# FAST-ASR/MarkovModels.jl

Measured on AMD Instinct MI355X. Metric: pdfposteriors_frames_per_sec, higher is better.
Workload: dtype f32

## Files before the change

### markovmodels.jl_amd/csrc/mm_engine.hip

```cpp
#include <hip/hip_runtime.h>
#include <dlfcn.h>

#include <algorithm>
#include <atomic>
#include <cmath>
#include <cstdio>
#include <cstdlib>
#include <chrono>
#include <cstring>
#include <limits>
#include <new>
#include <map>
#include <memory>
#include <mutex>
#include <string>
#include <thread>
#include <vector>

#include "../../include/markovmodels_amd.h"
#include "mm_kernels.hip"
#include "mm_kernel_quad.hip"
#include "mm_kernel_rows.hip"
#include "mm_internal.h"
#include "mm_pack.h"
// ... 2248 lines not shown
            "32-bit values), mm_stream_combine_kernel, mm_stream_finish_kernel, then for marked utterances only " + redo;
    case Fb::Split: {
        const std::string k = std::to_string(mm_pair_nj(h->max_P1, h->pair_H)), H = std::to_string(h->pair_H);
        return "mm_fbs_kernel<" + k + ",A," + H + ">, then <" + k + ",B," + H + "> (forward and backward agents in one grid, teams of " + H +
            " workgroups), mm_pair_finish_kernel, then for marked utterances only " +
            (h->dpair_ok ? "mm_fbds_kernel<" + k + ",A," + H + ">, then <" + k + ",B," + H + "> (float64, one utterance per team" +
                               (h->wpair_ok ? std::string("); FIRST and alone while the inputs are hard: mm_fbws_kernel<") + k + ",A," + H + ">, then <" + k +
                                                  ",B," + H + "> (wide-exponent pairs, two utterances per team)"
                                            : std::string("; FIRST and alone while the inputs are hard)")) +
                               ", mm_dpair_finish_kernel, then for what those mark "
                         : std::string()) +
            pair_tail;
    }
    case Fb::Pairs: {
        const std::string k = std::to_string(mm_pair_nj(h->max_P1));
        return "mm_fbp_kernel<" + k + ",A>, then <" + k + ",B> (forward and backward agents in one grid), mm_pair_finish_kernel, then for marked "
            "utterances only " +
            (h->dpair_ok ? "mm_fbd_kernel<" + k + ",A>, then <" + k + ",B> (float64, one utterance per workgroup" +
                               (h->wpair_ok ? std::string("); FIRST and alone while the inputs are hard: mm_fbw_kernel<") + k + ",A>, then <" + k +
                                                  ",B> (wide-exponent pairs, two utterances per workgroup)"
                                            : std::string("; FIRST and alone while the inputs are hard)")) +
                               ", mm_dpair_finish_kernel, then for what those mark "
                         : std::string()) +
            pair_tail;
    }
    case Fb::Rows: {
        auto ka = [&](int d) {
            for (int k : kRowKA)
                if (h->row_ka[d] <= k) return k;
            return 0;
        };
        return "mm_fbr_kernel<" + std::to_string(ka(0)) + ",8192,0> + mm_fbr_kernel<" + std::to_string(ka(1)) +
// ... 48 lines not shown
        const std::string inst = "<" + std::to_string(pl.NI) + "," + where_of(pl.global) + ">";
        s = "mm_leaky_fwd_kernel" + inst + " (forward: alpha~ with the leak term in the row epilogue) + mm_leaky_bwd_kernel" + inst +
            " (backward: z, then beta = z (+) eps c, gamma per pdf); state vectors " + (pl.global ? "in global memory" : "in LDS");
    } else if (entry == 2) {
        s = h->gen.last_kernels.empty() ? std::string("mm_generic_kernel (not called yet)") : h->gen.last_kernels;
    } else {
        return fail(MM_ERR_INVALID, "mm_batch_kernels: unknown entry");
    }
    snprintf(buf, n, "%s", s.c_str());
    return MM_OK;
}

static size_t ws_c_bytes(mm_batch_t h, int64_t N) { return align_up(size_t(h->B + 1) * size_t(N + 2) * 8, 256); }

struct WsLayout {
    size_t alpha = 0, c = 0, order = 0, redo = 0, hand = 0, zmin = 0, x = 0, x_rows = 0, xd = 0, xd_rows = 0, redo2 = 0;
    size_t extra = 0, em_max = 0, stream[4] = {0, 0, 0, 0}, total = 0;
};

static WsLayout ws_layout(mm_batch_t h, int64_t N) {
    WsLayout L;
    const size_t B = size_t(h->B), marks = align_up((B + 1) * 4, 256);
    L.c = on_pairs(h) ? align_up((B + 1) * size_t(h->pair_H > 1 ? h->split_s1p : h->max_S1p) * size_t(N + 2) * 4 + 16384, 256)
                      : align_up(size_t(h->total_s1p) * size_t(N + 1) * 4, 256);
    L.order = L.c + ws_c_bytes(h, N);
    L.redo = L.order + marks;
    L.hand = L.redo + marks;
    L.zmin = L.hand + align_up((B + 1) * 2 * mm_pair_hand_bytes(), 256);
    L.x = L.zmin + align_up(B * 6 * 8, 256);
    L.xd = L.redo2 = L.x;
    if (h->pair_H > 1) {
        const size_t H = size_t(h->pair_H), row = 2 * size_t(h->split_s1p) * 4, xps = size_t(mm_pair_xps(h->max_P1, h->pair_H)) * 4;
        L.x_rows = 2 * ((B + 1) / 2) * 2 * H * 2 * row;
        L.xd = L.redo2 = L.x + align_up(L.x_rows + ((B + 1) / 2) * 2 * H * 4 * xps, 256);
        if (h->dpair_ok) {
            L.xd_rows = 2 * B * 2 * H * 2 * row;
            L.redo2 = L.xd + align_up(L.xd_rows + B * 2 * H * 4 * xps + 65536, 256);
        }
    }
    L.extra = L.redo2 + marks;
    L.total = L.extra;
    if (h->fb == Fb::Stream) {
        L.total += mm_stream_extra_bytes(h->B, h->total_s1p, N, L.stream, h->stream_H, h->stream_S1);
        for (size_t &o : L.stream) o += L.extra;
// ... 194 lines not shown
        }
    }
    return launch_log<MODE_FB>(h, p, stream);
}

static int fb_linear(mm_batch_t h, RunParams &p, char *ws, const WsLayout &L, bool exact_first, void *stream) {
    h->last_redo = p.redo;
    h->last_exact_first = exact_first;
    int rc;
    if (h->fb == Fb::Rows) {
        rc = launch_rows(h, p, stream);
    } else {
        p.pair_s1p = h->pair_H > 1 ? h->split_s1p : h->max_S1p;
        p.pair_hand = ws + L.hand;
        p.pair_zmin = reinterpret_cast<double *>(ws + L.zmin);
        if (h->fb == Fb::Split) {
            p.xbuf_d = reinterpret_cast<float *>(ws + L.xd);
            p.xps_d = reinterpret_cast<float *>(ws + L.xd + L.xd_rows);
            p.x_phase_d = (long long)(L.xd_rows / 8);
            p.x_H = h->dpair_ok ? h->pair_H : 0;
            rc = bind_team_x(h, p, ws, L, exact_first, stream);
            if (rc) return rc;
        }
        h->last_z = p.pair_zmin;
        rc = exact_first ? MM_OK : launch_pairs(h, p, stream);
    }
    if (rc) return rc;
    if (h->dbg.no_redo && !exact_first) return MM_OK;
    if (h->dpair_ok) {
        const PairLaunch pl = pair_launch_of(h);
// ... 43 lines not shown
        if (h->dpair_ok) {
            const int64_t M = h->stat_host[0], H = h->pair_H, cus = std::max(1, h->n_cus);
            auto rounds = [&](int64_t wgs) { return (wgs + cus - 1) / cus; };
            const bool by_rounds = M > 0 && (h->wpair_ok || rounds(2 * h->B * H) <= rounds(2 * ((h->B + 1) / 2) * H) + rounds(2 * std::min<int64_t>(M, h->B) * H));
            exact_first = h->exact_first >= 0 ? h->exact_first != 0 : (by_rounds && !capturing(stream));
            p.redo2 = reinterpret_cast<int *>(ws + L.redo2);
            p.stat_dev = h->stat_dev;
            p.stat_xcd = h->xcd_counting ? 1 : 0;
            p.stat_host = h->stat_host;
            p.stat_seq = ++h->stat_seq;
            p.stat_mode = exact_first ? 1 : 0;
        }
    }
    if (ordered || marks) {
        hipLaunchKernelGGL(mm_prologue_kernel, dim3(unsigned((h->B + 1 + 255) / 256)), dim3(256), 0, static_cast<hipStream_t>(stream),
                           lens, int(h->B), int(N), order, p.redo, p.redo2, exact_first ? 1 : 0);
        HIP_TRY(hipGetLastError());
    }
    bind_stamps(h, p);
    switch (h->fb) {
    case Fb::Lane: return fb_lane(h, p, ws, L, stream);
    case Fb::Stream: return fb_stream(h, p, ws, L, stream);
    case Fb::Wave: return fb_wave(h, p, ws, L, stream);
    case Fb::Rows:
    case Fb::Pairs:
    case Fb::Split: return fb_linear(h, p, ws, L, exact_first, stream);
    case Fb::Quad:
    case Fb::Item: break;
    }
    return fb_exact(h, p, ws, L, stream);
}
// ... 344 lines not shown
        const WsLayout L = ws_layout(h, N);
        rc = ensure_ws(h, L.total, stream);
        if (rc) return rc;
        char *const ws = static_cast<char *>(h->ws);
        p.ws_alpha = reinterpret_cast<float *>(ws + L.alpha);
        p.ws_c = reinterpret_cast<double *>(ws + L.c);
        p.redo = reinterpret_cast<int *>(ws + L.redo);
        p.pair_s1p = h->pair_H > 1 ? h->split_s1p : h->max_S1p;
        p.pair_hand = ws + L.hand;
        p.pair_zmin = reinterpret_cast<double *>(ws + L.zmin);
        p.split_q10 = 512;
        p.lt_floor = h->lt_floor;
        p.x_sleep = h->dbg.x_sleep;
        p.x_timeout = x_timeout(N);
        hipLaunchKernelGGL(mm_prologue_kernel, dim3(unsigned((h->B + 1 + 255) / 256)), dim3(256), 0, static_cast<hipStream_t>(stream),
                           (const int *)nullptr, int(h->B), int(N), (int *)nullptr, p.redo, (int *)nullptr, 0);
        HIP_TRY(hipGetLastError());
        if (h->pair_H > 1) {
            rc = bind_team_x(h, p, ws, L, false, stream);
            if (rc) return rc;
            rc = mm_launch_split_export(pair_launch_of(h), p, mode == MODE_ALPHA ? 0 : 1, static_cast<hipStream_t>(stream));
        } else {
            rc = mm_launch_pair_export(pair_launch_of(h), p, mode == MODE_ALPHA ? 0 : 1, static_cast<hipStream_t>(stream));
        }
        if (rc) return rc;
        if (h->stat_host) {
            hipLaunchKernelGGL(mm_count_marks_kernel, dim3(1), dim3(256), 0, static_cast<hipStream_t>(stream), p.redo, int(h->B),
                               const_cast<int *>(h->stat_host) + 2 + (mode == MODE_ALPHA ? 0 : 1));
            HIP_TRY(hipGetLastError());
        }
        h->last_redo = p.redo;
// ... 173 lines not shown
```

### markovmodels.jl_amd/csrc/mm_kernel_dpair.hip

```cpp
#pragma once
#include "mm_kernel_pairs.hip"

namespace mm {

__device__ __forceinline__ double ldsr_d(unsigned addr) { return *(__attribute__((address_space(3))) const double *)(__UINTPTR_TYPE__)addr; }
__device__ __forceinline__ void ldsw_d(unsigned addr, double v) { *(__attribute__((address_space(3))) double *)(__UINTPTR_TYPE__)addr = v; }

__device__ __forceinline__ double dexp2(float y) {
    float fl = __builtin_floorf(y);
    fl = __builtin_fmaxf(fl, -1100.f);
    const float m = fast_exp2(y - fl);
    return __builtin_amdgcn_ldexp((double)m, (int)fl);
}
__device__ __forceinline__ float dlog2(double s) {
    const int ex = __builtin_amdgcn_frexp_exp(s);
    const float mf = (float)__builtin_amdgcn_frexp_mant(s);
    return (float)ex + fast_log2(mf);
}

#ifndef MM_DPAIR_LINFIN
#define MM_DPAIR_LINFIN 1
#endif
#define MM_DLINF_EMIN (-500.f)
template <int NJ>
// ... 857 lines not shown
            if (t1 > t0)
                dpair_pdf_sums<(NJ > 4 ? 1 : (NJ > 2 ? 2 : 3))>(L::Q(t1 & 1), L::PDFSE, L::PSUM(t1 & 1), P1, wave, NWC, lane, H > 1 ? xps_send + (t1 & 3) * (int)L::XPS : nullptr,
                               H > 1 && split_tag(t1, t0, 2) != 0u);
            __syncthreads();
        }
    }
#ifdef MM_STAMPS
    if (p.dbg && lane == 0 && H == 1)
        for (int k = 0; k < 2; ++k) p.dbg[(((long long)ui * MM_MAX_WAVES + wave) * 4 + PHASE * 2 + DIR) * 2 + k] = stamp_acc[k];
#endif
}

static __global__ void mm_dpair_finish_kernel(RunParams p) {
    const int b = blockIdx.x;
    if (p.redo[b] == 0) {
        if (p.stat_mode == 1 && threadIdx.x == 0) report_hard(p, 0);
        return;
    }
    int len = p.lens ? p.lens[b] : p.N;
    len = len < 0 ? 0 : (len > p.N ? p.N : len);
    const int P = p.utts[b].P1 - 1;
    if (threadIdx.x == 0) {
        const double z0 = p.pair_zmin[6 * b], z1 = p.pair_zmin[6 * b + 1];
        const double z = z0 < z1 ? z0 : z1;
        const double y0 = p.pair_zmin[6 * b + 2], y1 = p.pair_zmin[6 * b + 3];
        const double zM = y0 > y1 ? y0 : y1;
        const double l0 = p.pair_zmin[6 * b + 4], l1 = p.pair_zmin[6 * b + 5];
        const double lm = l0 < l1 ? l0 : l1;
        p.ttl[b] = (z < __builtin_inf()) ? (float)(z * (double)MM_LN2) : MM_NINF;
        const bool agree = z > -__builtin_inf() && zM < __builtin_inf() && zM - z <= MM_Z_SPREAD_TOL;
        if (p.redo2[b] == 1 && agree && lm >= (double)p.lt_floor - (double)MM_DPAIR_THR_EXTRA) p.redo2[b] = 0;
        if (p.redo2[b] == 0 && len >= 1 && !(zM < __builtin_inf())) p.redo2[b] = 1;
        if (p.redo2[b] == 0 && len >= 1 && !(z == -__builtin_inf() && zM == -__builtin_inf()) && !(lm >= (double)p.lt_floor - (double)MM_DPAIR_THR_EXTRA)) p.redo2[b] = 1;
        if (p.stat_mode == 1) report_hard(p, !(lm >= (double)p.lt_floor));
    }
    const long long gbase = (long long)b * p.gsb;
    for (long long q = threadIdx.x; q < (long long)(p.N - len) * P; q += blockDim.x)
        p.gamma[gbase + (len + q / P) * p.gsn + (q % P) * p.gsp] = 0.f;
}

}
```

### markovmodels.jl_amd/csrc/mm_kernel_pairs.hip

```cpp
#pragma once
#include <algorithm>
#include "mm_internal.h"
#include "mm_kernel_rows.hip"

namespace mm {

typedef float mm_f32x2 __attribute__((ext_vector_type(2)));
typedef unsigned mm_u32x2 __attribute__((ext_vector_type(2)));
__device__ __forceinline__ mm_u32x2 ldsr2u(unsigned addr) { return *(__attribute__((address_space(3))) const mm_u32x2 *)(__UINTPTR_TYPE__)addr; }
__device__ __forceinline__ mm_f32x2 ldsr2(unsigned addr) { return *(__attribute__((address_space(3))) const mm_f32x2 *)(__UINTPTR_TYPE__)addr; }
__device__ __forceinline__ void ldsw2(unsigned addr, float a, float b) {
    mm_f32x2 v = {a, b};
    *(__attribute__((address_space(3))) mm_f32x2 *)(__UINTPTR_TYPE__)addr = v;
}

constexpr int pair_pc(int NJ) { return NJ > 4 ? 64 * NJ : 256; }
constexpr int pair_nr(int RS, int PC) { return (PC > 256 || RS > 16384) ? 2 : 3; }
template <int RS, int PHASE, int RSH = 2 * RS, int PC = 256>
struct PairLay {
    static constexpr unsigned RS2 = 2 * RS;
    static constexpr unsigned PC4 = 4u * PC, PC8 = 8u * PC;
    static constexpr int NR = pair_nr(RS, PC);
    static constexpr unsigned RAWS = 2u * PC4;
    static constexpr unsigned XPS = 2u * PC;
// ... 614 lines not shown
    M(0) M(2) M(4) M(6) MM_PAIR_PRIO(MM_PAIR_PRIO_A, 1) M(8) M(10) M(12)                                     \
    if (lastp >= 14) {                                                                                       \
        M(14) MM_PAIR_PRIO(MM_PAIR_PRIO_B, 0) M(16)                                                          \
        if (lastp >= 18) {                                                                                   \
            M(18)                                                                                            \
            if (lastp >= 20) { M(20) M(22) }                                                                 \
        }                                                                                                    \
    }

struct PairHand {
    float m_prev, s_cur, s_prev, cbar;
    int seen, pad;
    double cum;
};

template <int KA, int RS, int PHASE, int DIRT, int NJ, int H = 1, int RSH = 2 * RS, bool SMALL = false, bool XPT = false>
__device__ __forceinline__ void pair_agent(const RunParams &p, int pair, int hset = 0, int rdir = 0) {
#ifndef MM_SPLIT_MAXTRACK
#define MM_SPLIT_MAXTRACK 0
#endif
    extern __shared__ float lds[];
    const int DIR = DIRT < 0 ? __builtin_amdgcn_readfirstlane(rdir) : DIRT;
    const unsigned long long x_tmo = p.x_timeout;
    using L = PairLay<RS, PHASE, RSH, pair_pc(NJ)>;
#ifndef MM_PAIR_DA
#define MM_PAIR_DA 3
#endif
#ifndef MM_PAIR_DB
#define MM_PAIR_DB 3
#endif
#ifndef MM_PAIR_EXITS_B
#define MM_PAIR_EXITS_B 1
// ... 30 lines not shown
    float *rowsP = p.ws_alpha + (long long)pair * (long long)(p.N + 2) * 2 * p.pair_s1p;
    const UttDesc &ud = p.utts[U[0].b];
    const RowU r = uni(H > 1 ? ud.rps[DIR][hset] : ud.rp[DIR]);
    const int S1 = r.rows, S1p = p.pair_s1p, P1 = uni(ud.P1), P = P1 - 1, P1p = (P1 + 3) & ~3;
    const float thr = r.thr;
    unsigned sthr = 0u;
    if constexpr (LINF && !ADAPT)
        asm volatile("v_readfirstlane_b32 %0, %1" : "=s"(sthr) : "v"(((unsigned)(127 - (int)(thr + MM_LINF_EMIN < 1.f ? 1.f : thr + MM_LINF_EMIN)) << 23) - 1u));
    int m = (int)(((long long)NFp * (p.split_q10 > 0 ? p.split_q10 : 512)) >> 10);
    m = m < 1 ? 1 : (m > NFp - 1 && NFp > 1 ? NFp - 1 : m);
    const int tA = XPT ? NFp : (DIR ? NFp - m : m), tEnd = NFp;
    auto frame_of = [&](int t) { return DIR ? NFp + 1 - t : t; };
    PairHand *hand = reinterpret_cast<PairHand *>(p.pair_hand) + ((long long)pair * 2 + DIR) * 2;
    if (lds_addr_of(lds) != 0u) __builtin_trap();
    MM_STAMP_DECL;

    for (unsigned q = tid * 4u; q < 2u * L::RS2; q += NT * 4u) ldsw(L::PP(0) + q, 0.f);
    if constexpr (PHASE == 1)
        for (unsigned q = tid * 4u; q < 2u * RSH; q += NT * 4u) ldsw(L::Q(0) + q, 0.f);
    if (tid < 32) ldsw(L::MS(0) + 4u * tid, 0.f);
    if (tid < 4) ldswu(L::MX(0) + 4u * tid, 0u);
    if (tid < 4) ldsw(L::EM(tid >> 1) + 8u * P1p + 4u * (tid & 1), LINF ? 0.f : MM_NINF);
    const int nslotwords = r.nslotrows * 128;
    for (int q = tid; q < nslotwords; q += NT) ldswu(L::SLOTS + 4u * q, as_global(r.slots)[q]);
    if constexpr (PHASE == 1)
        for (int q = tid; q < P1; q += NT) ldswu(L::PDFSE + 4u * q, as_global(reinterpret_cast<const unsigned *>(r.pdfse))[q]);
    int *redo0 = p.redo + U[0].b, *redo1 = p.redo + (U[1].valid ? U[1].b : p.B);
    const int xbase = H > 1 ? p.sp_base[hset] : 0, xcnt = H > 1 ? p.sp_cnt[hset] : 0;
    float *xsend = nullptr, *xps_send = nullptr;
    bool xplain = false;
// ... 121 lines not shown
                    }
                }
                if (sl == 0) ldswu(L::MS(t & 1), ((unsigned)(127 - (int)room) << 23) - 1u);
            }
            if (sl == 0) {
                if constexpr (!LINF) ldsw2(L::MS(t & 1), S[0], S[1]);
#pragma unroll
                for (int u = 0; u < 2; ++u) {
                    const double off = LINF ? cum[u] : (DIR ? cum[u] - (double)E[u] : cum[u]);
                    *(__attribute__((address_space(3))) double *)(__UINTPTR_TYPE__)(L::OWN(t & 3) + 8u * u) = LINF ? before[u] : off;
                    if (PHASE == 0) U[u].offs[frame_of(t)] = (XPT && DIR) ? before[u] : off;
                }
            }
        };
        for (int t = t0; t <= t0 + 3; ++t) dma_raw(t);
        if constexpr (PHASE == 1) {
            dma_partner(t0 + 1);
            if constexpr (L::NR == 3) dma_partner(t0 + 2);
#pragma unroll
            for (int u = 0; u < 2; ++u) {
                const PairHand h = hand[u];
                norm[u].m_prev = h.m_prev;
                norm[u].s_cur = h.s_cur;
                norm[u].s_prev = h.s_prev;
                norm[u].cbar = h.cbar;
                norm[u].seen = h.seen;
                cum[u] = h.cum;
            }
        }
        MM_ROW_VMCNT(0);
        if (PHASE == 0 || (DIR == 1 && !LINF)) {
            float E[2];
#pragma unroll
            for (int u = 0; u < 2; ++u) E[u] = pair_stage_em<NJ>(L::EM(t0 & 1), L::RAW(0, u) + L::RAWS * (unsigned)(t0 & 3), u, frame_of(t0), U[u].len, P, sl);
            if (PHASE == 0) {
#pragma unroll
                for (int u = 0; u < 2; ++u) cum[u] = (double)E[u];
                if (DIR == 0 && sl == 0) {
                    U[0].offs[1] = cum[0];
                    U[1].offs[1] = cum[1];
                }
            }
        }
        __syncthreads();
        if (t0 + 1 <= t1) {
            const float S[2] = {norm[0].s_cur, norm[1].s_cur};
            stage(t0 + 1, S);
        }
        dma_raw(t0 + 4);
        __syncthreads();
        const bool gwide = p.gsp == 1 && ((p.gsn | p.gsb) & 1) == 0 && ((__UINTPTR_TYPE__)p.gamma & 7) == 0;
        auto frames_of_step = [&](int ts, unsigned psum) {
            const int f = frame_of(ts);
            const bool live0 = f >= 1 && f <= U[0].len, live1 = f >= 1 && f <= U[1].len;
            float lt[2];
            const float *xp[H];
#pragma unroll
            for (int g = 0; g < H; ++g) xp[g] = (H > 1 && g != hset) ? xps_recv[g] + (ts & 3) * (int)L::XPS : nullptr;
            const bool writer = H == 1 || hset == 0;
// ... 248 lines not shown
                if (k == 0) __syncthreads();
                if (t > t0 && hset == 0) xframes(t, L::PSUM(t & 1));
            }
            if (lane == 0 && hset == 0) {
#pragma unroll
                for (int u = 0; u < 2; ++u)
                    if (U[u].valid) {
                        p.pair_zmin[(long long)U[u].b * 6 + DIR] = xzmin[u];
                        p.pair_zmin[(long long)U[u].b * 6 + 2 + DIR] = xzmax[u];
                        p.pair_zmin[(long long)U[u].b * 6 + 4 + DIR] = (double)xltmin[u];
                    }
            }
        }
    } else {
        __syncthreads();
        if (PHASE == 0 && DIR == 0) {
            for (int i = tid; i < S1; i += 64 * NWC) {
                unsigned pdfi = as_global(r.rowpdf)[i];
                if (H > 1 && pdfi == 0xffffu) pdfi = (unsigned)P1p;
                const unsigned e8 = 8u * pdfi;
                const mm_f32x2 e = ldsr2(L::EM(1) + e8);
                const float a = as_global(r.init)[i];
                float v0 = a + e.x, v1 = a + e.y;
                if (LINF && H > 1 && pdfi == (unsigned)P1p) v0 = v1 = MM_NINF;
                if (row_out_of_range(v0, thr)) *redo0 = 1;
                if (row_out_of_range(v1, thr)) *redo1 = 1;
                ldsw2(L::PP(1) + 8u * i, fast_exp2(v0), fast_exp2(v1));
                if constexpr (LINF) *reinterpret_cast<mm_f32x2 *>(rowsP + ((long long)1 * S1p + i) * 2) = mm_f32x2{fast_exp2(v0), fast_exp2(v1)};
                else *reinterpret_cast<mm_f32x2 *>(rowsP + ((long long)1 * S1p + i) * 2) = mm_f32x2{v0, v1};
            }
// ... 9 lines not shown
                    if (H > 1 && pdfi == 0xffffu) v0 = v1 = 0.f;
                    ldsw2(L::PP(t0 & 1) + 8u * i, v0, v1);
                    continue;
                }
                if (DIR == 1) {
                    const mm_f32x2 e = ldsr2(L::EM(t0 & 1) + 8u * (H > 1 && pdfi == 0xffffu ? (unsigned)P1p : pdfi));
                    v0 += e.x;
                    v1 += e.y;
                }
                if (H > 1 && pdfi == 0xffffu) v0 = v1 = MM_NINF;
                ldsw2(L::PP(t0 & 1) + 8u * i, fast_exp2(v0), fast_exp2(v1));
            }
        }
        load_graph();
        __syncthreads();
        if constexpr (H > 1) xplain = __builtin_amdgcn_readfirstlane(ldsru(L::XFLAG)) != 0u;
        bool cdead = H > 1 && (p.x_sleep & 0x200) != 0;
        auto step = [&](auto RDc, int t) {
            constexpr int RD = decltype(RDc)::value, WR = 1 - RD;
            float vmx0 = 0.f, vmx1 = 0.f;
            if (nslots > 0) {
                constexpr unsigned rdoff = L::PP(RD);
                mm_f32x2 x[2 * D];
#pragma unroll
                for (int j = 0; j < D; ++j) {
                    x[2 * j] = ldsr2(rg.a[(2 * j < KA) ? 2 * j : 0] + rdoff);
                    x[2 * j + 1] = ldsr2(rg.a[(2 * j + 1 < KA) ? 2 * j + 1 : 0] + rdoff);
                }
                unsigned sa = slot_base;
                unsigned info, info2 = 0u, infoN, info2N = 0u;
// ... 213 lines not shown
                }
            }
            MM_STAMP(0);
            MM_STEP_SYNC();
            MM_STAMP(1);
        };
        MM_STAMP_RESET;
        for (int t = t0 + 1; t <= t1; t += 2) {
            if (t & 1) step(std::integral_constant<int, 0>{}, t);
            else step(std::integral_constant<int, 1>{}, t);
            if (t + 1 <= t1) {
                if ((t + 1) & 1) step(std::integral_constant<int, 0>{}, t + 1);
                else step(std::integral_constant<int, 1>{}, t + 1);
            }
        }
        if constexpr (PHASE == 1) {
            if (t1 > t0)
                pair_pdf_sums<(NJ > 4 ? 1 : (NJ > 2 ? 2 : 3))>(L::Q(t1 & 1), L::PDFSE, L::PSUM(t1 & 1), P1, wave, NWC, lane, H > 1 ? xps_send + (t1 & 3) * (int)L::XPS : nullptr,
                              (H > 1 && split_tag(t1, t0, 2)) ? -1.f : 1.f);
            __syncthreads();
        }
    }
#ifdef MM_STAMPS
    if (p.dbg && lane == 0)
        for (int k = 0; k < 2; ++k) p.dbg[(((long long)pair * MM_MAX_WAVES + wave) * 4 + PHASE * 2 + DIR) * 2 + k] = stamp_acc[k];
    if (p.dbg && lane == 0 && service)
        for (int k = 0; k < 8; ++k)
            p.dbg[(long long)((p.B + 1) / 2) * MM_MAX_WAVES * 8 + ((long long)pair * 4 + PHASE * 2 + DIR) * 8 + k] = stamp_acc[k];
#endif
}

#ifndef MM_Z_SPREAD_TOL
#define MM_Z_SPREAD_TOL 2e-4
#define MM_LT_FLOOR (-20.0)
#endif
static __global__ void mm_pair_finish_kernel(RunParams p) {
    const int b = blockIdx.x;
    int len = p.lens ? p.lens[b] : p.N;
    len = len < 0 ? 0 : (len > p.N ? p.N : len);
    const int P = p.utts[b].P1 - 1;
    if (threadIdx.x == 0) {
        const double z0 = p.pair_zmin[6 * b], z1 = p.pair_zmin[6 * b + 1];
        const double z = z0 < z1 ? z0 : z1;
        const double y0 = p.pair_zmin[6 * b + 2], y1 = p.pair_zmin[6 * b + 3];
        const double zM = y0 > y1 ? y0 : y1;
        const double l0 = p.pair_zmin[6 * b + 4], l1 = p.pair_zmin[6 * b + 5];
        const double lm = l0 < l1 ? l0 : l1;
        p.ttl[b] = (z < __builtin_inf()) ? (float)(z * (double)MM_LN2) : MM_NINF;
        int mark = p.redo[b];
        const bool sound = z > -__builtin_inf() && zM < __builtin_inf() && zM - z <= MM_Z_SPREAD_TOL && lm >= (double)p.lt_floor;
        if (mark == 1 && sound && p.clear_marks) p.redo[b] = mark = 0;
        if (MM_PAIR_LINFIN && mark == 0 && len >= 1 && !(zM < __builtin_inf())) p.redo[b] = mark = 1;
        if (mark == 0 && len >= 1 && !(z == -__builtin_inf() && zM == -__builtin_inf()) && !(lm >= (double)p.lt_floor)) p.redo[b] = mark = 1;
        if (p.stat_mode == 0) report_hard(p, mark != 0);
    }
    const long long gbase = (long long)b * p.gsb;
    for (long long q = threadIdx.x; q < (long long)(p.N - len) * P; q += blockDim.x)
        p.gamma[gbase + (len + q / P) * p.gsn + (q % P) * p.gsp] = 0.f;
    if (p.x_H > 0 && p.xbuf_d) {
        __shared__ int marked;
        __syncthreads();
        if (threadIdx.x == 0) marked = p.redo[b];
        __syncthreads();
        if (marked) {
            typedef float f4 __attribute__((ext_vector_type(4)));
            const long long nrow = 2ll * p.x_H * 2 * p.x_slot, nps = 2ll * p.x_H * 4 * p.x_psn;
            for (int ph = 0; ph < 2; ++ph) {
                f4 *q = reinterpret_cast<f4 *>(p.xbuf_d + ph * p.x_phase_d + (long long)b * nrow);
                for (long long i = threadIdx.x; i < nrow / 4; i += blockDim.x) q[i] = f4{0.f, 0.f, 0.f, 0.f};
            }
            f4 *q = reinterpret_cast<f4 *>(p.xps_d + (long long)b * nps);
            for (long long i = threadIdx.x; i < nps / 4; i += blockDim.x) q[i] = f4{0.f, 0.f, 0.f, 0.f};
        }
// ... 96 lines not shown
```

### markovmodels.jl_amd/csrc/mm_kernels.hip

```cpp
#pragma once
#include <hip/hip_runtime.h>
#include <stdint.h>

#include <type_traits>

#include "mm_pack.h"

namespace mm {

#define MM_NINF (-__builtin_inff())
#define MM_LOG2E 1.4426950408889634f
#define MM_LN2 0.6931471805599453f
#define MM_MAX_WAVES 16
#define MM_SPLIT_HMAX 8

enum { MODE_FB = 0, MODE_ALPHA = 1, MODE_BETA = 2 };

struct GraphDev {
    const ItemMeta *items;
    const RowInfo *rowinfo;
    const Slot *slots;
    int n_items;
    int n_short;
};
// ... 74 lines not shown
    float *score;
    unsigned long long *dbg;
    int free_run;
    int xcsr;
    const int *order;
    int *redo;
    int *redo2;
    int *stat_dev;
    int clear_marks;
    volatile int *stat_host;
    int stat_seq, stat_mode;
    int stat_xcd;
    int pair_s1p;
    void *pair_hand;
    double *pair_zmin;
    int sp_base[MM_SPLIT_HMAX], sp_cnt[MM_SPLIT_HMAX];
    float *xbuf, *xps;
    long long x_slot, x_phase;
    float *xbuf_d, *xps_d;
    long long x_phase_d;
    int x_H;
    int split_q10;
    int x_psn;
    int x_sleep;
    unsigned long long x_timeout;
    float lt_floor;
    float g_scale;
    int g_acc;
    unsigned *sx;
    long long sx_slot;
};

__device__ __forceinline__ void report_hard(const RunParams &p, int hard) {
    if (!p.stat_dev) return;
    atomicAdd(&p.stat_dev[0], hard);
    __threadfence();
    if (atomicAdd(&p.stat_dev[1], 1) == (int)gridDim.x - 1) {
        __threadfence();
        const int total = atomicAdd(&p.stat_dev[0], 0);
        p.stat_dev[0] = 0;
        p.stat_dev[1] = 0;
        p.stat_host[0] = total;
        p.stat_host[1] = p.stat_seq;
        __threadfence_system();
    }
}

#ifdef MM_STAMPS
#define MM_STAMP(slot)                                                                     \
    do {                                                                                   \
        unsigned long long t_;                                                             \
        __builtin_amdgcn_sched_barrier(0);                                                 \
// ... 851 lines not shown
__global__ void mm_pick_final_kernel(const UttDesc *utts, int B, const float *A, long long stride_n, int n, float *out) {
    const int b = blockIdx.x * blockDim.x + threadIdx.x;
    if (b < B) out[b] = A[(long long)n * stride_n + utts[b].state_off + utts[b].S1 - 1];
}

__global__ void mm_maxmarginal_kernel(const UttDesc *utts, float *A, long long a_stride_n, const float *Bt, long long b_stride_n,
                                      const float *best) {
    const int b = blockIdx.x, n = blockIdx.y;
    const UttDesc &u = utts[b];
    const float bb = best[b];
    float *a = A + (long long)n * a_stride_n + u.state_off;
    const float *bt = Bt + (long long)n * b_stride_n + u.state_off;
    for (int s = threadIdx.x; s < u.S1; s += blockDim.x) a[s] = (bb > MM_NINF) ? a[s] + bt[s] - bb : MM_NINF;
}

__global__ void __launch_bounds__(256) mm_prologue_kernel(const int *lens, int B, int N, int *order, int *redo, int *redo2, int fill) {
    __shared__ int sh[256];
    const int i = blockIdx.x * blockDim.x + threadIdx.x;
    if (i <= B) {
        if (redo) redo[i] = i < B ? fill : 0;
        if (redo2) redo2[i] = 0;
    }
    if (!lens || !order) return;
    auto clamp = [&](int l) { return l < 0 ? 0 : (l > N ? N : l); };
    const int li = i < B ? clamp(lens[i]) : 0;
    int rank = 0;
    for (int j0 = 0; j0 < B; j0 += 256) {
        __syncthreads();
        sh[threadIdx.x] = j0 + (int)threadIdx.x < B ? clamp(lens[j0 + threadIdx.x]) : -1;
        __syncthreads();
        const int n = B - j0 < 256 ? B - j0 : 256;
        for (int k = 0; k < n; ++k) {
            const int lj = sh[k], j = j0 + k;
            rank += (lj > li) || (lj == li && j < i);
        }
    }
// ... 62 lines not shown
```

### markovmodels.jl_amd/csrc/mm_pairs_tu.hip

```cpp
#define MM_SECONDARY_TU
#include "mm_internal.h"
#include "mm_kernel_pairs.hip"

namespace mm {

template <int NJ, int PHASE, bool SMALL>
__global__ void __launch_bounds__(1024) mm_fbp_kernel(RunParams p) {
    const int npairs = (p.B + 1) / 2, dir = (int)blockIdx.x >= npairs;
    pair_agent<MM_PAIR_KA, MM_ROW_RS, PHASE, -1, NJ, 1, 2 * MM_ROW_RS, SMALL>(p, (int)blockIdx.x - (dir ? npairs : 0), 0, dir);
}
template <int NJ, int PHASE, bool SMALL>
static int launch_pair_phase(const PairLaunch &pl, const RunParams &p, hipStream_t st) {
    return pair_launch_phase(mm_fbp_kernel<NJ, PHASE, SMALL>, "pair kernel", pair_lds_bytes(MM_ROW_RS, PHASE, pl.slotrows, 0, pair_pc(NJ)),
                             2 * pair_count(pl), pl.nwc + 1, st, p);
}
template <int NJ, bool SMALL>
static int launch_pairs_ka(const PairLaunch &pl, const RunParams &p, hipStream_t s0) {
    return pair_launch_phases(launch_pair_phase<NJ, 0, SMALL>, launch_pair_phase<NJ, 1, SMALL>, mm_pair_finish_kernel, pl, p, s0);
}
int mm_launch_pairs(const PairLaunch &pl, const RunParams &p, hipStream_t s0) {
    if (pl.pair_ka > MM_PAIR_KA) return MM_ERR_UNSUPPORTED;
    if (pl.max_P1 <= 128) return pl.small ? launch_pairs_ka<2, true>(pl, p, s0) : launch_pairs_ka<2, false>(pl, p, s0);
    if (pl.max_P1 <= 250) return launch_pairs_ka<4, false>(pl, p, s0);
    if (pl.max_P1 > MM_PAIR_P1MAX) return MM_ERR_UNSUPPORTED;
    return launch_pairs_ka<8, false>(pl, p, s0);
}
template <int NJ, bool SMALL>
__global__ void __launch_bounds__(1024) mm_fbx_kernel(RunParams p, int dir) {
    pair_agent<MM_PAIR_KA, MM_ROW_RS, 0, -1, NJ, 1, 2 * MM_ROW_RS, SMALL, true>(p, (int)blockIdx.x, 0, dir);
}
template <int NJ, bool SMALL>
static int launch_pair_export(const PairLaunch &pl, const RunParams &p, int dir, hipStream_t st) {
    const int rc = pair_launch_phase(mm_fbx_kernel<NJ, SMALL>, "pair kernel", pair_lds_bytes(MM_ROW_RS, 0, pl.slotrows, 0, pair_pc(NJ)), pair_count(pl),
                                     pl.nwc + 1, st, p, dir);
    return rc ? rc : pair_launch_export_layout(pl, p, dir, st);
}
bool mm_pair_export_fits(const PairLaunch &pl) { return pl.H == 1 && pl.pair_ka <= MM_PAIR_KA && pl.max_P1 <= 250; }
int mm_launch_pair_export(const PairLaunch &pl, const RunParams &p, int dir, hipStream_t s0) {
    if (!mm_pair_export_fits(pl)) return MM_ERR_UNSUPPORTED;
    if (pl.max_P1 <= 128) return pl.small ? launch_pair_export<2, true>(pl, p, dir, s0) : launch_pair_export<2, false>(pl, p, dir, s0);
// ... 9 lines not shown
```

Baseline: 146.1 million.

## Fuse pair phases A, B and finish into one launch with per-pair flags

For pair kernels with NJ up to 4, the forward/backward phase A, phase B and the finish kernel now run in one launch. The two agents of a pair sit in neighbouring workgroups and hand phase A over through a global flag with release/acquire fences and a timed spin-wait. Whichever agent arrives last runs the finish decision, and zeroing of the gamma tail moves between the phases. This removes two kernel launches and the grid-wide barriers between phases. It relies on both agents of a pair being co-resident, and falls back to marking utterances for redo if the wait times out.

```diff
diff --git a/markovmodels.jl_amd/csrc/mm_engine.hip b/markovmodels.jl_amd/csrc/mm_engine.hip
--- a/markovmodels.jl_amd/csrc/mm_engine.hip
+++ b/markovmodels.jl_amd/csrc/mm_engine.hip
@@ -2286,8 +2286,10 @@
     }
     case Fb::Pairs: {
         const std::string k = std::to_string(mm_pair_nj(h->max_P1));
-        return "mm_fbp_kernel<" + k + ",A>, then <" + k + ",B> (forward and backward agents in one grid), mm_pair_finish_kernel, then for marked "
-            "utterances only " +
+        return (mm_pair_nj(h->max_P1) > 4
+                    ? "mm_fbp_kernel<" + k + ",A>, then <" + k + ",B> (forward and backward agents in one grid), mm_pair_finish_kernel, then for marked utterances only "
+                    : "mm_fbp_kernel<" + k + "> (both phases in one launch: the forward and the backward agent of a pair as neighbouring workgroups in one grid, "
+            "phase A handed over per pair, the pair's finish by whichever agent arrives last), then for marked utterances only ") +
             (h->dpair_ok ? "mm_fbd_kernel<" + k + ",A>, then <" + k + ",B> (float64, one utterance per workgroup" +
                                (h->wpair_ok ? std::string("); FIRST and alone while the inputs are hard: mm_fbw_kernel<") + k + ",A>, then <" + k +
                                                   ",B> (wide-exponent pairs, two utterances per workgroup)"
@@ -2366,7 +2368,7 @@
 static size_t ws_c_bytes(mm_batch_t h, int64_t N) { return align_up(size_t(h->B + 1) * size_t(N + 2) * 8, 256); }
 
 struct WsLayout {
-    size_t alpha = 0, c = 0, order = 0, redo = 0, hand = 0, zmin = 0, x = 0, x_rows = 0, xd = 0, xd_rows = 0, redo2 = 0;
+    size_t alpha = 0, c = 0, order = 0, redo = 0, hand = 0, zmin = 0, psync = 0, x = 0, x_rows = 0, xd = 0, xd_rows = 0, redo2 = 0;
     size_t extra = 0, em_max = 0, stream[4] = {0, 0, 0, 0}, total = 0;
 };
 
@@ -2379,7 +2381,8 @@
     L.redo = L.order + marks;
     L.hand = L.redo + marks;
     L.zmin = L.hand + align_up((B + 1) * 2 * mm_pair_hand_bytes(), 256);
-    L.x = L.zmin + align_up(B * 6 * 8, 256);
+    L.psync = L.zmin + align_up(B * 6 * 8, 256);
+    L.x = L.psync + align_up(((B + 1) / 2) * 16, 256);
     L.xd = L.redo2 = L.x;
     if (h->pair_H > 1) {
         const size_t H = size_t(h->pair_H), row = 2 * size_t(h->split_s1p) * 4, xps = size_t(mm_pair_xps(h->max_P1, h->pair_H)) * 4;
@@ -2604,6 +2607,7 @@
         p.pair_s1p = h->pair_H > 1 ? h->split_s1p : h->max_S1p;
         p.pair_hand = ws + L.hand;
         p.pair_zmin = reinterpret_cast<double *>(ws + L.zmin);
+        p.pair_sync = reinterpret_cast<unsigned *>(ws + L.psync);
         if (h->fb == Fb::Split) {
             p.xbuf_d = reinterpret_cast<float *>(ws + L.xd);
             p.xps_d = reinterpret_cast<float *>(ws + L.xd + L.xd_rows);
@@ -2677,7 +2681,8 @@
     }
     if (ordered || marks) {
         hipLaunchKernelGGL(mm_prologue_kernel, dim3(unsigned((h->B + 1 + 255) / 256)), dim3(256), 0, static_cast<hipStream_t>(stream),
-                           lens, int(h->B), int(N), order, p.redo, p.redo2, exact_first ? 1 : 0);
+                           lens, int(h->B), int(N), order, p.redo, p.redo2, exact_first ? 1 : 0,
+                           h->fb == Fb::Pairs ? reinterpret_cast<unsigned *>(ws + L.psync) : (unsigned *)nullptr);
         HIP_TRY(hipGetLastError());
     }
     bind_stamps(h, p);
@@ -3052,7 +3057,7 @@
         p.x_sleep = h->dbg.x_sleep;
         p.x_timeout = x_timeout(N);
         hipLaunchKernelGGL(mm_prologue_kernel, dim3(unsigned((h->B + 1 + 255) / 256)), dim3(256), 0, static_cast<hipStream_t>(stream),
-                           (const int *)nullptr, int(h->B), int(N), (int *)nullptr, p.redo, (int *)nullptr, 0);
+                           (const int *)nullptr, int(h->B), int(N), (int *)nullptr, p.redo, (int *)nullptr, 0, (unsigned *)nullptr);
         HIP_TRY(hipGetLastError());
         if (h->pair_H > 1) {
             rc = bind_team_x(h, p, ws, L, false, stream);
diff --git a/markovmodels.jl_amd/csrc/mm_kernel_dpair.hip b/markovmodels.jl_amd/csrc/mm_kernel_dpair.hip
--- a/markovmodels.jl_amd/csrc/mm_kernel_dpair.hip
+++ b/markovmodels.jl_amd/csrc/mm_kernel_dpair.hip
@@ -895,7 +895,7 @@
 static __global__ void mm_dpair_finish_kernel(RunParams p) {
     const int b = blockIdx.x;
     if (p.redo[b] == 0) {
-        if (p.stat_mode == 1 && threadIdx.x == 0) report_hard(p, 0);
+        if (p.stat_mode == 1 && threadIdx.x == 0) report_hard(p, 0, (int)gridDim.x);
         return;
     }
     int len = p.lens ? p.lens[b] : p.N;
@@ -913,7 +913,7 @@
         if (p.redo2[b] == 1 && agree && lm >= (double)p.lt_floor - (double)MM_DPAIR_THR_EXTRA) p.redo2[b] = 0;
         if (p.redo2[b] == 0 && len >= 1 && !(zM < __builtin_inf())) p.redo2[b] = 1;
         if (p.redo2[b] == 0 && len >= 1 && !(z == -__builtin_inf() && zM == -__builtin_inf()) && !(lm >= (double)p.lt_floor - (double)MM_DPAIR_THR_EXTRA)) p.redo2[b] = 1;
-        if (p.stat_mode == 1) report_hard(p, !(lm >= (double)p.lt_floor));
+        if (p.stat_mode == 1) report_hard(p, !(lm >= (double)p.lt_floor), (int)gridDim.x);
     }
     const long long gbase = (long long)b * p.gsb;
     for (long long q = threadIdx.x; q < (long long)(p.N - len) * P; q += blockDim.x)
diff --git a/markovmodels.jl_amd/csrc/mm_kernel_pairs.hip b/markovmodels.jl_amd/csrc/mm_kernel_pairs.hip
--- a/markovmodels.jl_amd/csrc/mm_kernel_pairs.hip
+++ b/markovmodels.jl_amd/csrc/mm_kernel_pairs.hip
@@ -652,8 +652,29 @@
     double cum;
 };
 
-template <int KA, int RS, int PHASE, int DIRT, int NJ, int H = 1, int RSH = 2 * RS, bool SMALL = false, bool XPT = false>
-__device__ __forceinline__ void pair_agent(const RunParams &p, int pair, int hset = 0, int rdir = 0) {
+typedef __attribute__((address_space(1))) unsigned mm_gu32;
+__device__ __forceinline__ mm_gu32 *pair_sync_word(unsigned *w) { return (mm_gu32 *)(__UINTPTR_TYPE__)w; }
+__device__ __forceinline__ bool pair_publish() {
+    asm volatile("s_waitcnt vmcnt(0)" ::: "memory");
+    __syncthreads();
+    if (threadIdx.x != 0) return false;
+    __builtin_amdgcn_fence(__ATOMIC_RELEASE, "agent");
+    asm volatile("s_waitcnt vmcnt(0)" ::: "memory");
+    return true;
+}
+__device__ __forceinline__ bool pair_wait_flag(unsigned *flag, unsigned long long tmo) {
+    const unsigned long long tstart = __builtin_amdgcn_s_memrealtime();
+    for (;;) {
+        const unsigned v = __hip_atomic_load(pair_sync_word(flag), __ATOMIC_RELAXED, __HIP_MEMORY_SCOPE_AGENT);
+        if (__builtin_amdgcn_readfirstlane((int)v) != 0) return true;
+        if (__builtin_amdgcn_s_memrealtime() - tstart > tmo) return false;
+        __builtin_amdgcn_s_sleep(8);
+    }
+}
+
+template <int KA, int RS, int PHASE, int DIRT, int NJ, int H = 1, int RSH = 2 * RS, bool SMALL = false, bool XPT = false, bool FUSED = false>
+__device__ __forceinline__ bool pair_agent(const RunParams &p, int pair, int hset = 0, int rdir = 0) {
+    static_assert(!FUSED || (H == 1 && !XPT), "the one-launch form is the pairs' proper");
 #ifndef MM_SPLIT_MAXTRACK
 #define MM_SPLIT_MAXTRACK 0
 #endif
@@ -714,6 +735,19 @@
     PairHand *hand = reinterpret_cast<PairHand *>(p.pair_hand) + ((long long)pair * 2 + DIR) * 2;
     if (lds_addr_of(lds) != 0u) __builtin_trap();
     MM_STAMP_DECL;
+#ifdef MM_STAMPS
+    unsigned long long *const stamp_abs =
+        p.dbg ? p.dbg + (long long)((p.B + 1) / 2) * (MM_MAX_WAVES * 8 + 32) + ((long long)pair * 4 + PHASE * 2 + DIR) * 4 : nullptr;
+#define MM_STAMP_ABS(k)                                                                  \
+    do {                                                                                 \
+        if (stamp_abs && tid == 0) stamp_abs[k] = __builtin_amdgcn_s_memrealtime();      \
+    } while (0)
+#else
+#define MM_STAMP_ABS(k) \
+    do {                \
+    } while (0)
+#endif
+    MM_STAMP_ABS(0);
 
     for (unsigned q = tid * 4u; q < 2u * L::RS2; q += NT * 4u) ldsw(L::PP(0) + q, 0.f);
     if constexpr (PHASE == 1)
@@ -865,9 +899,24 @@
             }
         };
         for (int t = t0; t <= t0 + 3; ++t) dma_raw(t);
+        bool fdead = false;
+        if constexpr (PHASE == 1 && FUSED) {
+            unsigned *const flag = p.pair_sync + 4ll * pair + (1 - DIR);
+            fdead = (p.x_sleep & 0x1000) != 0 || !pair_wait_flag(flag, x_tmo);
+            if (!fdead) {
+                __builtin_amdgcn_fence(__ATOMIC_ACQUIRE, "agent");
+                asm volatile("s_waitcnt vmcnt(0)" ::: "memory");
+            } else if (sl == 0) {
+                *redo0 = 2;
+                *redo1 = 2;
+            }
+            if (sl == 0) ldswu(L::XFLAG, fdead ? 1u : 0u);
+        }
         if constexpr (PHASE == 1) {
-            dma_partner(t0 + 1);
-            if constexpr (L::NR == 3) dma_partner(t0 + 2);
+            if (!fdead) {
+                dma_partner(t0 + 1);
+                if constexpr (L::NR == 3) dma_partner(t0 + 2);
+            }
 #pragma unroll
             for (int u = 0; u < 2; ++u) {
                 const PairHand h = hand[u];
@@ -894,6 +943,7 @@
             }
         }
         __syncthreads();
+        if (FUSED && fdead) return false;
         if (t0 + 1 <= t1) {
             const float S[2] = {norm[0].s_cur, norm[1].s_cur};
             stage(t0 + 1, S);
@@ -1172,6 +1222,8 @@
         }
     } else {
         __syncthreads();
+        if constexpr (PHASE == 1 && FUSED)
+            if (__builtin_amdgcn_readfirstlane((int)ldsru(L::XFLAG)) != 0) return false;
         if (PHASE == 0 && DIR == 0) {
             for (int i = tid; i < S1; i += 64 * NWC) {
                 unsigned pdfi = as_global(r.rowpdf)[i];
@@ -1211,6 +1263,7 @@
         }
         load_graph();
         __syncthreads();
+        MM_STAMP_ABS(1);
         if constexpr (H > 1) xplain = __builtin_amdgcn_readfirstlane(ldsru(L::XFLAG)) != 0u;
         bool cdead = H > 1 && (p.x_sleep & 0x200) != 0;
         auto step = [&](auto RDc, int t) {
@@ -1454,6 +1507,7 @@
                 else step(std::integral_constant<int, 1>{}, t + 1);
             }
         }
+        MM_STAMP_ABS(2);
         if constexpr (PHASE == 1) {
             if (t1 > t0)
                 pair_pdf_sums<(NJ > 4 ? 1 : (NJ > 2 ? 2 : 3))>(L::Q(t1 & 1), L::PDFSE, L::PSUM(t1 & 1), P1, wave, NWC, lane, H > 1 ? xps_send + (t1 & 3) * (int)L::XPS : nullptr,
@@ -1468,35 +1522,50 @@
         for (int k = 0; k < 8; ++k)
             p.dbg[(long long)((p.B + 1) / 2) * MM_MAX_WAVES * 8 + ((long long)pair * 4 + PHASE * 2 + DIR) * 8 + k] = stamp_acc[k];
 #endif
+    MM_STAMP_ABS(3);
+    return true;
 }
 
 #ifndef MM_Z_SPREAD_TOL
 #define MM_Z_SPREAD_TOL 2e-4
 #define MM_LT_FLOOR (-20.0)
 #endif
+__device__ __forceinline__ bool pair_finish_decide(const RunParams &p, int b, int len) {
+    typedef __attribute__((address_space(1))) double mm_gf64;
+    auto zld = [&](int k) {
+        return __hip_atomic_load((mm_gf64 *)(__UINTPTR_TYPE__)(p.pair_zmin + 6ll * b + k), __ATOMIC_RELAXED, __HIP_MEMORY_SCOPE_AGENT);
+    };
+    {
+        const double z0 = zld(0), z1 = zld(1);
+        const double z = z0 < z1 ? z0 : z1;
+        const double y0 = zld(2), y1 = zld(3);
+        const double zM = y0 > y1 ? y0 : y1;
+        const double l0 = zld(4), l1 = zld(5);
+        const double lm = l0 < l1 ? l0 : l1;
+        p.ttl[b] = (z < __builtin_inf()) ? (float)(z * (double)MM_LN2) : MM_NINF;
+        int mark = (int)__hip_atomic_load(pair_sync_word(reinterpret_cast<unsigned *>(p.redo + b)), __ATOMIC_RELAXED, __HIP_MEMORY_SCOPE_AGENT);
+        const bool sound = z > -__builtin_inf() && zM < __builtin_inf() && zM - z <= MM_Z_SPREAD_TOL && lm >= (double)p.lt_floor;
+        if (mark == 1 && sound && p.clear_marks) p.redo[b] = mark = 0;
+        if (MM_PAIR_LINFIN && mark == 0 && len >= 1 && !(zM < __builtin_inf())) p.redo[b] = mark = 1;
+        if (mark == 0 && len >= 1 && !(z == -__builtin_inf() && zM == -__builtin_inf()) && !(lm >= (double)p.lt_floor)) p.redo[b] = mark = 1;
+        return mark != 0;
+    }
+}
+__device__ __forceinline__ void pair_zero_tail(const RunParams &p, int b, int len, int P) {
+    const long long gbase = (long long)b * p.gsb;
+    for (long long q = threadIdx.x; q < (long long)(p.N - len) * P; q += blockDim.x)
+        p.gamma[gbase + (len + q / P) * p.gsn + (q % P) * p.gsp] = 0.f;
+}
 static __global__ void mm_pair_finish_kernel(RunParams p) {
     const int b = blockIdx.x;
     int len = p.lens ? p.lens[b] : p.N;
     len = len < 0 ? 0 : (len > p.N ? p.N : len);
     const int P = p.utts[b].P1 - 1;
     if (threadIdx.x == 0) {
-        const double z0 = p.pair_zmin[6 * b], z1 = p.pair_zmin[6 * b + 1];
-        const double z = z0 < z1 ? z0 : z1;
-        const double y0 = p.pair_zmin[6 * b + 2], y1 = p.pair_zmin[6 * b + 3];
-        const double zM = y0 > y1 ? y0 : y1;
-        const double l0 = p.pair_zmin[6 * b + 4], l1 = p.pair_zmin[6 * b + 5];
-        const double lm = l0 < l1 ? l0 : l1;
-        p.ttl[b] = (z < __builtin_inf()) ? (float)(z * (double)MM_LN2) : MM_NINF;
-        int mark = p.redo[b];
-        const bool sound = z > -__builtin_inf() && zM < __builtin_inf() && zM - z <= MM_Z_SPREAD_TOL && lm >= (double)p.lt_floor;
-        if (mark == 1 && sound && p.clear_marks) p.redo[b] = mark = 0;
-        if (MM_PAIR_LINFIN && mark == 0 && len >= 1 && !(zM < __builtin_inf())) p.redo[b] = mark = 1;
-        if (mark == 0 && len >= 1 && !(z == -__builtin_inf() && zM == -__builtin_inf()) && !(lm >= (double)p.lt_floor)) p.redo[b] = mark = 1;
-        if (p.stat_mode == 0) report_hard(p, mark != 0);
-    }
-    const long long gbase = (long long)b * p.gsb;
-    for (long long q = threadIdx.x; q < (long long)(p.N - len) * P; q += blockDim.x)
-        p.gamma[gbase + (len + q / P) * p.gsn + (q % P) * p.gsp] = 0.f;
+        const bool marked = pair_finish_decide(p, b, len);
+        if (p.stat_mode == 0) report_hard(p, marked, (int)gridDim.x);
+    }
+    pair_zero_tail(p, b, len, P);
     if (p.x_H > 0 && p.xbuf_d) {
         __shared__ int marked;
         __syncthreads();
diff --git a/markovmodels.jl_amd/csrc/mm_kernels.hip b/markovmodels.jl_amd/csrc/mm_kernels.hip
--- a/markovmodels.jl_amd/csrc/mm_kernels.hip
+++ b/markovmodels.jl_amd/csrc/mm_kernels.hip
@@ -112,6 +112,7 @@
     int pair_s1p;
     void *pair_hand;
     double *pair_zmin;
+    unsigned *pair_sync;
     int sp_base[MM_SPLIT_HMAX], sp_cnt[MM_SPLIT_HMAX];
     float *xbuf, *xps;
     long long x_slot, x_phase;
@@ -129,11 +130,11 @@
     long long sx_slot;
 };
 
-__device__ __forceinline__ void report_hard(const RunParams &p, int hard) {
+__device__ __forceinline__ void report_hard(const RunParams &p, int hard, int expected) {
     if (!p.stat_dev) return;
     atomicAdd(&p.stat_dev[0], hard);
     __threadfence();
-    if (atomicAdd(&p.stat_dev[1], 1) == (int)gridDim.x - 1) {
+    if (atomicAdd(&p.stat_dev[1], 1) == expected - 1) {
         __threadfence();
         const int total = atomicAdd(&p.stat_dev[0], 0);
         p.stat_dev[0] = 0;
@@ -1015,12 +1016,14 @@
     for (int s = threadIdx.x; s < u.S1; s += blockDim.x) a[s] = (bb > MM_NINF) ? a[s] + bt[s] - bb : MM_NINF;
 }
 
-__global__ void __launch_bounds__(256) mm_prologue_kernel(const int *lens, int B, int N, int *order, int *redo, int *redo2, int fill) {
+__global__ void __launch_bounds__(256) mm_prologue_kernel(const int *lens, int B, int N, int *order, int *redo, int *redo2, int fill,
+                                                          unsigned *psync) {
     __shared__ int sh[256];
     const int i = blockIdx.x * blockDim.x + threadIdx.x;
     if (i <= B) {
         if (redo) redo[i] = i < B ? fill : 0;
         if (redo2) redo2[i] = 0;
+        if (psync && 2 * i < 4 * ((B + 1) / 2)) psync[2 * i] = psync[2 * i + 1] = 0u;
     }
     if (!lens || !order) return;
     auto clamp = [&](int l) { return l < 0 ? 0 : (l > N ? N : l); };
diff --git a/markovmodels.jl_amd/csrc/mm_pairs_tu.hip b/markovmodels.jl_amd/csrc/mm_pairs_tu.hip
--- a/markovmodels.jl_amd/csrc/mm_pairs_tu.hip
+++ b/markovmodels.jl_amd/csrc/mm_pairs_tu.hip
@@ -4,26 +4,73 @@
 
 namespace mm {
 
+typedef __attribute__((address_space(4))) const RunParams mm_kparams;
+__device__ __forceinline__ const RunParams &pair_params() {
+    mm_kparams *k = (mm_kparams *)__builtin_amdgcn_kernarg_segment_ptr();
+    asm volatile("" : "+s"(k));
+    return *(const RunParams *)k;
+}
+template <int NJ, bool SMALL>
+__global__ void __launch_bounds__(1024) mm_fbp_kernel(RunParams) {
+    const int pair = (int)blockIdx.x >> 1, dir = (int)blockIdx.x & 1;
+    bool absent;
+    {
+        const RunParams &p = pair_params();
+        absent = (p.x_sleep & 0x2000) != 0 && dir == 1;
+        if (!absent) {
+            pair_agent<MM_PAIR_KA, MM_ROW_RS, 0, -1, NJ, 1, 2 * MM_ROW_RS, SMALL, false, true>(p, pair, 0, dir);
+            if (pair_publish()) __hip_atomic_store(pair_sync_word(p.pair_sync + 4ll * pair + dir), 1u, __ATOMIC_RELAXED, __HIP_MEMORY_SCOPE_AGENT);
+        }
+    }
+    const RunParams &p = pair_params();
+    unsigned *const sync = p.pair_sync + 4ll * pair;
+    const int iu = 2 * pair + dir;
+    if (iu < p.B) {
+        const int b = p.order ? p.order[iu] : iu;
+        int len = p.lens ? p.lens[b] : p.N;
+        len = len < 0 ? 0 : (len > p.N ? p.N : len);
+        pair_zero_tail(p, b, len, p.utts[b].P1 - 1);
+    }
+    if (absent) {
+        if (threadIdx.x == 0)
+            for (int u = 0; u < 2; ++u) p.redo[2 * pair + u < p.B ? (p.order ? p.order[2 * pair + u] : 2 * pair + u) : p.B] = 2;
+    } else {
+        pair_agent<MM_PAIR_KA, MM_ROW_RS, 1, -1, NJ, 1, 2 * MM_ROW_RS, SMALL, false, true>(p, pair, 0, dir);
+    }
+    if (!pair_publish()) return;
+    if (__hip_atomic_fetch_add(pair_sync_word(sync + 2), 1u, __ATOMIC_RELAXED, __HIP_MEMORY_SCOPE_AGENT) != 1u) return;
+    __builtin_amdgcn_fence(__ATOMIC_ACQUIRE, "agent");
+    int hard = 0;
+    for (int u = 0; u < 2; ++u) {
+        if (2 * pair + u >= p.B) continue;
+        const int b = p.order ? p.order[2 * pair + u] : 2 * pair + u;
+        int len = p.lens ? p.lens[b] : p.N;
+        len = len < 0 ? 0 : (len > p.N ? p.N : len);
+        hard += pair_finish_decide(p, b, len) ? 1 : 0;
+    }
+    if (p.stat_mode == 0) report_hard(p, hard, (int)gridDim.x >> 1);
+}
+template <int NJ, bool SMALL>
+static int launch_pairs_ka(const PairLaunch &pl, const RunParams &p, hipStream_t s0) {
+    return pair_launch_phase(mm_fbp_kernel<NJ, SMALL>, "pair kernel", pair_lds_bytes(MM_ROW_RS, 1, pl.slotrows, 0, pair_pc(NJ)), 2 * pair_count(pl),
+                             pl.nwc + 1, s0, p);
+}
 template <int NJ, int PHASE, bool SMALL>
 __global__ void __launch_bounds__(1024) mm_fbp_kernel(RunParams p) {
     const int npairs = (p.B + 1) / 2, dir = (int)blockIdx.x >= npairs;
     pair_agent<MM_PAIR_KA, MM_ROW_RS, PHASE, -1, NJ, 1, 2 * MM_ROW_RS, SMALL>(p, (int)blockIdx.x - (dir ? npairs : 0), 0, dir);
 }
-template <int NJ, int PHASE, bool SMALL>
+template <int NJ, int PHASE>
 static int launch_pair_phase(const PairLaunch &pl, const RunParams &p, hipStream_t st) {
-    return pair_launch_phase(mm_fbp_kernel<NJ, PHASE, SMALL>, "pair kernel", pair_lds_bytes(MM_ROW_RS, PHASE, pl.slotrows, 0, pair_pc(NJ)),
+    return pair_launch_phase(mm_fbp_kernel<NJ, PHASE, false>, "pair kernel", pair_lds_bytes(MM_ROW_RS, PHASE, pl.slotrows, 0, pair_pc(NJ)),
                              2 * pair_count(pl), pl.nwc + 1, st, p);
-}
-template <int NJ, bool SMALL>
-static int launch_pairs_ka(const PairLaunch &pl, const RunParams &p, hipStream_t s0) {
-    return pair_launch_phases(launch_pair_phase<NJ, 0, SMALL>, launch_pair_phase<NJ, 1, SMALL>, mm_pair_finish_kernel, pl, p, s0);
 }
 int mm_launch_pairs(const PairLaunch &pl, const RunParams &p, hipStream_t s0) {
     if (pl.pair_ka > MM_PAIR_KA) return MM_ERR_UNSUPPORTED;
     if (pl.max_P1 <= 128) return pl.small ? launch_pairs_ka<2, true>(pl, p, s0) : launch_pairs_ka<2, false>(pl, p, s0);
     if (pl.max_P1 <= 250) return launch_pairs_ka<4, false>(pl, p, s0);
     if (pl.max_P1 > MM_PAIR_P1MAX) return MM_ERR_UNSUPPORTED;
-    return launch_pairs_ka<8, false>(pl, p, s0);
+    return pair_launch_phases(launch_pair_phase<8, 0>, launch_pair_phase<8, 1>, mm_pair_finish_kernel, pl, p, s0);
 }
 template <int NJ, bool SMALL>
 __global__ void __launch_bounds__(1024) mm_fbx_kernel(RunParams p, int dir) {
```

New measurement: 144.9 million. Within noise of the previous version (-0.8%).
